# Jaakk0F/DSTD-GCN

Measured on AMD Instinct MI355X. Metric: pose-sequences/sec forward (H36M 22J×50T, B=256) at 1/2/4/8 GPUs; % HBM roofline, higher is better.
Workload: dtype f32; 1 GPU; H36M-shape synthetic, T=10+25=35, V=22, B=256/GPU, eval forward; global_batch=256, seq_len=35, joints=22, parallelism=dp1

## Files before the change

### dstd-gcn_amd/csrc/dstd_capi.hip

```cpp
#include <stdlib.h>
#include <string.h>

#include <algorithm>

#include <vector>

#include "../../include/dstd_gcn.h"
#include "../../include/dstd_gcn_taps.h"
#include "dstd_common.h"
#include "dstd_hilo.h"
#include "dstd_kernels.h"
#include "dstd_taps.h"

using namespace dstd;

namespace {

constexpr int kMaxT = 128;
constexpr int kMaxV = 32;
constexpr int kMaxC = 64;

struct Carver {
  char* base;
  size_t off = 0;
// ... 854 lines not shown
                        const dstd_block_taps* taps, void* workspace, size_t workspace_bytes, void* stream,
                        unsigned flags) {
  if ((flags & ~DSTD_FWD_EXACT_FP32) || !taps) return DSTD_EINVAL;
  return block_fwd(p, x, B, T, V, y, workspace, workspace_bytes, stream, flags, taps);
}

}

namespace {

int block_fwd(const dstd_block_params* p, const float* x, int B, int T, int V, float* y, void* workspace,
              size_t workspace_bytes, void* stream, unsigned flags, const dstd_block_taps* taps) {
  StreamDeviceGuard dev_guard_(stream, x);
  if (!x || !y || !workspace || !block_ok(p) || !shape_ok(B, T, V)) return DSTD_EINVAL;
  if (!limits_ok(T, V, p->cin, p->cout)) return DSTD_ELIMIT;
  if (workspace_bytes < dstd_block_workspace_bytes(B, p->cin, p->cout, T, V)) return DSTD_EWORKSPACE;
  hipStream_t s = (hipStream_t)stream;
  Carver cv{(char*)workspace};
  BlockLayout L;
  carve_block(cv, L, B, p->cin, p->cout, T, V);
  FoldList fa;
  add_block_jobs(fa, p, L.f, T, V);
  DSTD_TRY(run_fold(fa, s));
  DSTD_TRY(to_layout(x, L.xin, B, p->cin, T * V, 1, s));
  DSTD_TRY(spatial_pq(p, L.xin, B, T, V, L.sc.pq_s, s));
  BlockTail tail{TEPI_RAW, nullptr, nullptr, nullptr, nullptr, nullptr};
  const BlockHL hl = block_hl(p, tail, B, T, V, flags, taps != nullptr);
  HLList hj;
  add_block_hl_jobs(hj, p, L.f, tail, hl, T, V);
  DSTD_TRY(run_hl_prep(hj, s));
  Prof pf;
  DSTD_TRY(run_block(p, L.f, L.sc, B, T, V, L.xin, L.h, L.yout, tail, s, pf, hl, nullptr, taps));
  DSTD_TRY(to_layout(L.yout, y, B, p->cout, T * V, 0, s));
  return DSTD_OK;
}

}

extern "C" {

int dstd_model_fwd(const dstd_model_params* p, const float* x, int B, float* y, void* workspace,
                   size_t workspace_bytes, void* stream) {
  return dstd_model_fwd_ex(p, x, B, y, workspace, workspace_bytes, stream, 0u, nullptr);
}

int dstd_model_fwd_profiled(const dstd_model_params* p, const float* x, int B, float* y, void* workspace,
                            size_t workspace_bytes, void* stream, dstd_profile* prof) {
  return dstd_model_fwd_ex(p, x, B, y, workspace, workspace_bytes, stream, 0u, prof);
}

int dstd_model_fwd_ex(const dstd_model_params* p, const float* x, int B, float* y, void* workspace,
                      size_t workspace_bytes, void* stream, unsigned flags, dstd_profile* prof) {
  if (flags & ~(DSTD_FWD_REUSE_CONSTANTS | DSTD_FWD_EXACT_FP32 | DSTD_FWD_SEPARATE_ADJ | DSTD_FWD_FUSED_TEMPORAL |
                DSTD_FWD_SEPARATE_BLOCK | DSTD_FWD_SEPARATE_ENCODERS))
    return DSTD_EINVAL;
  return model_fwd(p, x, B, y, workspace, workspace_bytes, stream, flags, prof, nullptr);
}

size_t dstd_model_taps_workspace_bytes(int B, int T, int V, int num_feature, int num_layers) {
  return dstd_model_workspace_bytes(B, T, V, num_feature, num_layers);
}

int dstd_model_fwd_taps(const dstd_model_params* p, const float* x, int B, float* y, const dstd_block_taps* taps,
                        void* workspace, size_t workspace_bytes, void* stream, unsigned flags) {
  if ((flags & ~DSTD_FWD_EXACT_FP32) || !taps) return DSTD_EINVAL;
  return model_fwd(p, x, B, y, workspace, workspace_bytes, stream, flags, nullptr, taps);
}

}

namespace {

int model_fwd(const dstd_model_params* p, const float* x, int B, float* y, void* workspace, size_t workspace_bytes,
              void* stream, unsigned flags, dstd_profile* prof, const dstd_block_taps* taps) {
  StreamDeviceGuard dev_guard_(stream, x);
  if (taps) flags |= DSTD_FWD_SEPARATE_ADJ | DSTD_FWD_SEPARATE_BLOCK | DSTD_FWD_SEPARATE_ENCODERS;
  const bool reuse = (flags & DSTD_FWD_REUSE_CONSTANTS) != 0;
  if (!p || !x || !y || !workspace) return DSTD_EINVAL;
  if (prof && (prof->capacity < 0 || (prof->capacity > 0 && (!prof->events || !prof->kinds)))) return DSTD_EINVAL;
  Prof pf;
  pf.p = prof;
  const int T = p->T, V = p->V, C = p->num_feature, L_ = p->num_layers;
  if (!shape_ok(B, T, V) || L_ < 0 || L_ > DSTD_MAX_LAYERS || p->in_channels != 6) return DSTD_EINVAL;
  if (!limits_ok(T, V, p->in_channels, C)) return DSTD_ELIMIT;
  if (!block_ok(&p->st_in) || !block_ok(&p->st_out) || !bn_ok(p->bn_in) || !p->prelu) return DSTD_EINVAL;
  if (p->st_in.cin != 6 || p->st_in.cout != C || p->st_out.cin != C || p->st_out.cout != 3) return DSTD_EINVAL;
  for (int i = 0; i < L_; ++i) {
    if (!block_ok(&p->enc[i]) || !bn_ok(p->enc_bn[i]) || !p->enc_prelu[i]) return DSTD_EINVAL;
    if (p->enc[i].cin != C || p->enc[i].cout != C) return DSTD_EINVAL;
  }
  if (workspace_bytes < dstd_model_workspace_bytes(B, T, V, C, L_)) return DSTD_EWORKSPACE;
  hipStream_t s = (hipStream_t)stream;
  Carver cv{(char*)workspace};
  ModelLayout L;
  carve_model(cv, L, B, T, V, C, L_, 6, 3);

  FoldList fa;
  add_block_jobs(fa, &p->st_in, L.f_in, T, V);
  add_block_jobs(fa, &p->st_out, L.f_out, T, V);
  add_bn_job(fa, p->bn_in, C, V, L.bnin_s, L.bnin_h);
  for (int i = 0; i < L_; ++i) {
    add_block_jobs(fa, &p->enc[i], L.f_enc[i], T, V);
    add_bn_job(fa, p->enc_bn[i], C, V, L.ebn_s[i], L.ebn_h[i]);
  }
  if (!reuse) {
    pf.begin(DSTD_KIND_FOLD, s);
    DSTD_TRY(run_fold(fa, s));
// ... 44 lines not shown
    hls[b] = block_hl(blk[b], tails[b], B, T, V, flags, taps != nullptr);
    add_block_hl_jobs(hj, blk[b], *fold[b], tails[b], hls[b], T, V);
  }
  for (int b = 1; b < NB && !(flags & DSTD_FWD_SEPARATE_ADJ); ++b)
    if (hls[b].s && hls[b - 1].tf && blk[b - 1]->cout == 64 && temporal_fused_phase3(T, V)) {
      hls[b].s_pre = true;
      tails[b - 1].next_f = fold[b];
      tails[b - 1].next_adj = true;
    }
  if (hls[0].bf && !(flags & DSTD_FWD_SEPARATE_ADJ) && blk[0]->cin == 6 && block_fused_adj0_supported(T, V))
    hls[0].adj0 = true;

  PQArgs pa{};
  pa.x = x;
  pa.B = B;
  pa.T = T;
  pa.V = V;
  pa.Cin = 6;
  pa.make_x6 = 1;
  pa.x6 = L.act[0];
  const dstd_block_params* b0 = &p->st_in;
  pa.w[0] = b0->conv_s[0].wm1;
  pa.w[1] = b0->conv_s[0].wm2;
  pa.w[2] = b0->conv_s[1].wm1;
  pa.w[3] = b0->conv_s[1].wm2;
  pa.b[0] = b0->conv_s[0].bm1;
  pa.b[1] = b0->conv_s[0].bm2;
  pa.b[2] = b0->conv_s[1].bm1;
  pa.b[3] = b0->conv_s[1].bm2;
  pa.nw = 4;
  pa.pq = L.sc.pq_s;
  pa.pql = pq_layout_vt(8, T, V);
  if (!hls[0].s || (taps && taps[0].x)) {
    pf.begin(DSTD_KIND_PREP, s);
    DSTD_TRY(launch_pq(pa, s));
    pf.end(s);
  }

  if (!reuse) {
    pf.begin(DSTD_KIND_FOLD, s);
    DSTD_TRY(run_hl_prep(hj, s));
    pf.end(s);
  }
  const bool chain = !(flags & (DSTD_FWD_SEPARATE_ENCODERS | DSTD_FWD_SEPARATE_BLOCK | DSTD_FWD_SEPARATE_ADJ)) &&
                     !(prof && prof->capacity > 0) && enc_chain_supported(T, V);
  auto chain_block = [&](int b, EncChainArgs* c) {
    if (!chain || b < 1 || b > L_ || !hls[b].bf || !hls[b].s_pre || !tails[b].next_adj) return false;
    BlockArgs A;
    build_block_args(A, blk[b], *fold[b], L.sc, B, T, V, xin[b], hbuf[b], ybuf[b], tails[b], hls[b], nullptr);
    BlockFusedArgs ba;
    return block_fused_args(A.ha, A.ht, A.aht, &A.sn, &ba, nullptr) == hipSuccess &&
           enc_chain_append(c, ba) == hipSuccess;
  };
  for (int b = 0; b < NB;) {
    EncChainArgs c{};
    int e = b;
    while (e < NB && chain_block(e, &c)) ++e;
    if (e - b >= 2) {
      DSTD_TRY(launch_enc_chain(c, s));
      b = e;
      continue;
    }
    pf.block = b;
    DSTD_TRY(run_block(blk[b], *fold[b], L.sc, B, T, V, xin[b], hbuf[b], ybuf[b], tails[b], s, pf, hls[b],
                       b == 0 ? x : nullptr, taps ? &taps[b] : nullptr));
    ++b;
  }
  return DSTD_OK;
}

}

extern "C" {


int dstd_events_create(int n, void** events) {
  if (n < 0 || (n > 0 && !events)) return DSTD_EINVAL;
  for (int i = 0; i < n; ++i) {
    hipEvent_t e;
    DSTD_TRY(hipEventCreate(&e));
    events[i] = (void*)e;
  }
  return DSTD_OK;
}

int dstd_events_destroy(int n, void** events) {
  if (n < 0 || (n > 0 && !events)) return DSTD_EINVAL;
  for (int i = 0; i < n; ++i)
    if (events[i]) DSTD_TRY(hipEventDestroy((hipEvent_t)events[i]));
  return DSTD_OK;
}

int dstd_event_elapsed_ms(void* start, void* stop, float* ms) {
  if (!start || !stop || !ms) return DSTD_EINVAL;
  return (int)hipEventElapsedTime(ms, (hipEvent_t)start, (hipEvent_t)stop);
}

}
```

### dstd-gcn_amd/csrc/dstd_hilo.h

```cpp
#pragma once
#include "dstd_common.h"
#include "dstd_kernels.h"

namespace dstd {

typedef _Float16 f16x8 __attribute__((ext_vector_type(8)));

typedef float f32x2_t __attribute__((ext_vector_type(2)));
typedef _Float16 f16x2_t __attribute__((ext_vector_type(2)));

__device__ __forceinline__ void split8(const float4& a, const float4& b, uint4& hi, uint4& lo) {
  hi.x = __builtin_bit_cast(uint32_t, __builtin_convertvector((f32x2_t){a.x, a.y}, f16x2_t));
  hi.y = __builtin_bit_cast(uint32_t, __builtin_convertvector((f32x2_t){a.z, a.w}, f16x2_t));
  hi.z = __builtin_bit_cast(uint32_t, __builtin_convertvector((f32x2_t){b.x, b.y}, f16x2_t));
  hi.w = __builtin_bit_cast(uint32_t, __builtin_convertvector((f32x2_t){b.z, b.w}, f16x2_t));
  asm("v_fma_mixlo_f16 %0, %4, 1.0, -%12 op_sel_hi:[0,0,1]\n\t"
      "v_fma_mixhi_f16 %0, %5, 1.0, -%12 op_sel:[0,0,1] op_sel_hi:[0,0,1]\n\t"
      "v_fma_mixlo_f16 %1, %6, 1.0, -%13 op_sel_hi:[0,0,1]\n\t"
      "v_fma_mixhi_f16 %1, %7, 1.0, -%13 op_sel:[0,0,1] op_sel_hi:[0,0,1]\n\t"
      "v_fma_mixlo_f16 %2, %8, 1.0, -%14 op_sel_hi:[0,0,1]\n\t"
      "v_fma_mixhi_f16 %2, %9, 1.0, -%14 op_sel:[0,0,1] op_sel_hi:[0,0,1]\n\t"
      "v_fma_mixlo_f16 %3, %10, 1.0, -%15 op_sel_hi:[0,0,1]\n\t"
      "v_fma_mixhi_f16 %3, %11, 1.0, -%15 op_sel:[0,0,1] op_sel_hi:[0,0,1]\n\t"
      "s_nop 1"
// ... 259 lines not shown
};
static_assert(sizeof(EncChainArgs) <= 4096, "kernel arguments end at 4 KB");
__host__ __device__ inline void enc_chain_apply(const EncChainDesc& d, SpatialHLArgs& s) {
  s.x = d.x;
  s.y = d.h;
  for (int g = 0; g < 2; ++g) {
    s.wimg[g] = d.s_wimg[g];
    s.wscale[g] = d.s_wscale[g];
    s.bf[g] = d.s_bf[g];
    s.adjb[g] = d.s_adjb[g];
    s.pqb[g] = d.s_pqb[g];
  }
  s.bn_s = d.s_bn_s;
  s.bn_h = d.s_bn_h;
  s.prelu = d.s_prelu;
  s.pqimg = d.s_pqimg;
  s.pqscale = d.s_pqscale;
}
__host__ __device__ inline void enc_chain_apply(const EncChainDesc& d, TemporalHLArgs& g) {
  g.h = d.h;
  g.wimg = d.t_wimg;
  g.wscale = d.t_wscale;
  g.bf = d.t_bf;
  g.adjb = d.t_adjb;
  g.xres = d.t_xres;
  g.bn_s = d.t_bn_s;
  g.bn_h = d.t_bn_h;
  g.prelu = d.t_prelu;
  g.y = d.y;
  g.pqimg = d.t_pqimg;
  g.pqscale = d.t_pqscale;
  for (int i = 0; i < 4; ++i) g.pqb[i] = d.t_pqb[i];
}
__host__ __device__ inline void enc_chain_apply_j(const EncChainDesc& d, AdjHLArgs& j) {
  j.wimg[0] = d.j_wimg;
  j.wscale[0] = d.j_wscale;
  j.bias[0] = d.j_bias;
  j.astat[0] = d.j_astat;
  j.alpha = d.j_alpha;
}
__host__ __device__ inline void enc_chain_apply_sn(const EncChainDesc& d, AdjHLArgs& sn) {
  for (int g = 0; g < 2; ++g) {
    sn.wimg[g] = d.n_wimg[g];
    sn.wscale[g] = d.n_wscale[g];
    sn.bias[g] = d.n_bias[g];
    sn.astat[g] = d.n_astat[g];
  }
  sn.alpha = d.n_alpha;
}
bool enc_chain_supported(int T, int V);
hipError_t enc_chain_append(EncChainArgs* c, const BlockFusedArgs& a);
hipError_t launch_enc_chain(const EncChainArgs& c, hipStream_t s);


}
```

### dstd-gcn_amd/csrc/dstd_hilo.hip

```cpp
#include <type_traits>

#include "dstd_common.h"
#include "dstd_hilo.h"
#include "dstd_kernels.h"

#ifdef DSTD_STAMPS
__device__ unsigned long long g_tl_hl[6][2048][4];
#define TLH(m, i) \
  if (threadIdx.x == 0 && blockIdx.x < 2048) g_tl_hl[m][blockIdx.x][i] = __builtin_amdgcn_s_memrealtime();
#else
#define TLH(m, i)
#endif

namespace dstd {

namespace {


__device__ __forceinline__ float4 ld4(const float* p) { return *reinterpret_cast<const float4*>(p); }
__device__ __forceinline__ f16x8 as_h8(const uint4& v) { return __builtin_bit_cast(f16x8, v); }
typedef _Float16 f16x4 __attribute__((ext_vector_type(4)));

__device__ __forceinline__ f32x4 mfma32(const f16x8& a, const f16x8& b, f32x4 c) {
  return __builtin_amdgcn_mfma_f32_16x16x32_f16(a, b, c, 0, 0, 0);
// ... 2210 lines not shown
  __device__ __forceinline__ KP base() const {
    KP p = (KP)__builtin_amdgcn_kernarg_segment_ptr();
    asm volatile("" : "+s"(p));
    return p;
  }
  template <typename S, typename P>
  __device__ __forceinline__ static S get(P p) {
    S r;
    __builtin_memcpy(&r, p, sizeof(S));
    return r;
  }
  __device__ __forceinline__ SpatialHLArgsVal s() const {
    KP p = base();
    SpatialHLArgsVal r = get<SpatialHLArgsVal>(&p->s);
    enc_chain_apply(get<EncChainDesc>(&p->enc[b]), r);
    return r;
  }
  __device__ __forceinline__ TemporalHLArgs tg() const {
    KP p = base();
    TemporalHLArgs r = get<TemporalHLArgs>(&p->t.g);
    enc_chain_apply(get<EncChainDesc>(&p->enc[b]), r);
    return r;
  }
  __device__ __forceinline__ AdjHLArgs tj() const {
    KP p = base();
    AdjHLArgs r = get<AdjHLArgs>(&p->t.j);
    enc_chain_apply_j(get<EncChainDesc>(&p->enc[b]), r);
    return r;
  }
  __device__ __forceinline__ AdjHLArgs tsn() const {
    KP p = base();
    AdjHLArgs r = get<AdjHLArgs>(&p->t.sn);
    enc_chain_apply_sn(get<EncChainDesc>(&p->enc[b]), r);
    return r;
  }
  __device__ __forceinline__ AdjHLArgs s0() const { return AdjHLArgs{}; }
  __device__ __forceinline__ static uint32_t zero() { return (uint32_t)opaque_zero(); }
};

template <int T, int V>
__global__ __launch_bounds__((64 * tf_waves<T, V>())) __attribute__((amdgpu_waves_per_eu((tf_waves<T, V>() / 4), (tf_waves<T, V>() / 4)))) void k_enc_chain(EncChainArgs ca) {
  extern __shared__ __attribute__((aligned(16))) unsigned char dsm[];
#pragma nounroll
  for (int b = 0; b < ca.nblk; ++b) {
    int tid = threadIdx.x, n = blockIdx.x, lds0 = 0;
    asm volatile("" : "+v"(tid));
    asm volatile("" : "+s"(n), "+s"(lds0));
    block_fused_body<T, V, 64, 64, TEPI_ENC>(EncChainArgsAt{b}, n, dsm + lds0, tid);
    __builtin_amdgcn_s_waitcnt(0);
    __syncthreads();
  }
}

namespace {

int hl_num_cus() {
  static int n = [] {
    int dev = 0, v = 0;
    if (hipGetDevice(&dev) != hipSuccess ||
        hipDeviceGetAttribute(&v, hipDeviceAttributeMultiprocessorCount, dev) != hipSuccess || v <= 0)
      v = 256;
    return v;
  }();
  return n;
}

template <typename K>
int hl_occupancy(K k, int nt) {
  int nb = 0;
  if (hipOccupancyMaxActiveBlocksPerMultiprocessor(&nb, (const void*)k, nt, 0) != hipSuccess || nb < 1) nb = 1;
  (void)hipGetLastError();
  return nb;
}

template <auto K, int NT, typename A>
hipError_t launch_units(int units, const A& a, hipStream_t s) {
  static const int occ = hl_occupancy(K, NT);
  int grid = hl_num_cus() * occ;
  grid = min(grid, cdiv(units, NT / 64));
  hipLaunchKernelGGL(K, dim3(grid), dim3(NT), 0, s, a);
  return hipGetLastError();
}

template <int T>
hipError_t temporal_hl_t(const TemporalHLArgs& a, hipStream_t s) {
  if (a.C == 3) {
    if (a.pq) return hipErrorNotSupported;
    switch (a.epi) {
      case TEPI_OUT: return launch_units<k_temporal_hl<T, TEPI_OUT, 3>, temporal_nt<T, 3>()>(a.B * a.V, a, s);
      case TEPI_RAW: return launch_units<k_temporal_hl<T, TEPI_RAW, 3>, temporal_nt<T, 3>()>(a.B * a.V, a, s);
      default: return hipErrorNotSupported;
    }
  }
  if (a.C != 64) return hipErrorNotSupported;
  switch (a.epi) {
    case TEPI_ENC:
      if constexpr (tf_res_acc(T, 25)) {
        if (a.V == 25) return launch_units<k_temporal_hl<T, TEPI_ENC, 64, true>, temporal_nt<T, 64>()>(a.B * a.V, a, s);
      }
      if constexpr (tf_res_acc(T, 23)) {
        if (a.V == 23) return launch_units<k_temporal_hl<T, TEPI_ENC, 64, true>, temporal_nt<T, 64>()>(a.B * a.V, a, s);
      }
      return launch_units<k_temporal_hl<T, TEPI_ENC, 64>, temporal_nt<T, 64>()>(a.B * a.V, a, s);
    case TEPI_IN: return launch_units<k_temporal_hl<T, TEPI_IN, 64>, temporal_nt<T, 64>()>(a.B * a.V, a, s);
    case TEPI_RAW: return launch_units<k_temporal_hl<T, TEPI_RAW, 64>, temporal_nt<T, 64>()>(a.B * a.V, a, s);
    default: return hipErrorNotSupported;
// ... 109 lines not shown

template <int T, int V>
hipError_t bfused_tv(const BlockFusedArgs& a, hipStream_t s) {
  const int cin = a.s.Cin, cout = a.s.Cout, epi = a.t.g.epi;
  if (cin == 64 && cout == 64 && epi == TEPI_ENC) return bfused_run<T, V, 64, 64, TEPI_ENC>(a, s);
  if (cin == 6 && cout == 64 && epi == TEPI_IN) return bfused_run<T, V, 6, 64, TEPI_IN>(a, s);
  if (cin == 64 && cout == 3 && epi == TEPI_OUT) return bfused_run<T, V, 64, 3, TEPI_OUT>(a, s);
  return hipErrorNotSupported;
}

bool block_fused_supported(int T, int V, int cin, int cout, int epi) {
  const bool shape = (T == 35 && (V == 22 || V == 25)) || (T == 40 && V == 23);
  return shape && ((cin == 64 && cout == 64 && epi == TEPI_ENC) || (cin == 6 && cout == 64 && epi == TEPI_IN) ||
                   (cin == 64 && cout == 3 && epi == TEPI_OUT));
}

bool block_fused_adj0_supported(int T, int V) {
  return block_fused_supported(T, V, 6, 64, TEPI_IN) && temporal_fused_phase3(T, V);
}

static bool phase3_args_ok(const TemporalHLArgs& g, const AdjHLArgs& sn) {
  return temporal_fused_phase3(g.T, g.V) && g.C == 64 && g.pq && sn.pq == g.pq && sn.ngroups == 2 && !sn.xin &&
         sn.pql.sch == 1 && !(sn.pql.st & 3) && !(sn.pql.sv & 3) && !(sn.pql.sn & 3) && !(sn.p_ch[0] & 3) &&
         !(sn.p_ch[1] & 3) && sn.out;
}

hipError_t block_fused_args(const SpatialHLArgs& sa, const TemporalHLArgs& g, const AdjHLArgs& j, const AdjHLArgs* sn,
                            BlockFusedArgs* out, const AdjHLArgs* s0) {
  if (!block_fused_supported(g.T, g.V, sa.Cin, sa.Cout, g.epi) || sa.T != g.T || sa.V != g.V || sa.B != g.B ||
      sa.Cout != g.C || sa.y != g.h || sa.pq != j.pq || g.V != (int)(j.pql.st / 4) || j.pql.sch != 1 || j.pql.sv != 4 ||
      ((uintptr_t)j.pq & 15) || j.p_ch[0] != 0 || j.pql.sn != (long)g.T * g.V * 4)
    return hipErrorNotSupported;
  if (sn && !phase3_args_ok(g, *sn)) return hipErrorNotSupported;
  if (s0 && (sa.Cin != 6 || !block_fused_adj0_supported(g.T, g.V) || !s0->xin || s0->ngroups != 2 || !s0->out ||
             s0->B != g.B || !sa.xmodel || sa.adj != s0->out))
    return hipErrorNotSupported;
  *out = BlockFusedArgs{sa, TemporalFusedArgs{g, j, sn ? *sn : AdjHLArgs{}}, s0 ? *s0 : AdjHLArgs{}};
  return hipSuccess;
}

hipError_t launch_block_fused(const SpatialHLArgs& sa, const TemporalHLArgs& g, const AdjHLArgs& j, const AdjHLArgs* sn,
                              hipStream_t s, const AdjHLArgs* s0) {
  BlockFusedArgs a;
  const hipError_t e = block_fused_args(sa, g, j, sn, &a, s0);
  if (e != hipSuccess) return e;
  if (g.T == 35 && g.V == 22) return bfused_tv<35, 22>(a, s);
  if (g.T == 35 && g.V == 25) return bfused_tv<35, 25>(a, s);
  if (g.T == 40 && g.V == 23) return bfused_tv<40, 23>(a, s);
  return hipErrorNotSupported;
}

bool enc_chain_supported(int T, int V) { return block_fused_supported(T, V, 64, 64, TEPI_ENC) && temporal_fused_phase3(T, V); }

hipError_t enc_chain_append(EncChainArgs* c, const BlockFusedArgs& a) {
  const SpatialHLArgs& s = a.s;
  const TemporalHLArgs& g = a.t.g;
  const AdjHLArgs &j = a.t.j, &n = a.t.sn;
  if (!enc_chain_supported(g.T, g.V) || s.Cin != 64 || s.Cout != 64 || g.epi != TEPI_ENC || s.xmodel || !n.out ||
      a.s0.out || g.xres != s.x || s.wimg[2] || s.wscale[2] || s.bf[2] || s.rbn_s || s.rbn_h || j.xin || n.xin)
    return hipErrorNotSupported;
  if (c->nblk == 0) {
    c->s = s;
    c->t = a.t;
  } else {
    const SpatialHLArgs& s0 = c->s;
    const TemporalHLArgs& g0 = c->t.g;
    const AdjHLArgs &j0 = c->t.j, &n0 = c->t.sn;
    auto same_adj = [](const AdjHLArgs& p, const AdjHLArgs& q) {
      return p.pq == q.pq && p.pql.sn == q.pql.sn && p.pql.st == q.pql.st && p.pql.sv == q.pql.sv &&
             p.pql.sch == q.pql.sch && p.p_ch[0] == q.p_ch[0] && p.p_ch[1] == q.p_ch[1] && p.B == q.B &&
             p.ngroups == q.ngroups && p.out == q.out && p.out_sN == q.out_sN && p.out_sG == q.out_sG &&
             p.nchunk == q.nchunk;
    };
    if (c->nblk >= kEncChainMax || s.B != s0.B || s.T != s0.T || s.V != s0.V || s.adj != s0.adj || s.pq != s0.pq ||
        g.B != g0.B || g.T != g0.T || g.V != g0.V || g.C != g0.C || g.adj != g0.adj || g.pq != g0.pq ||
        !same_adj(j, j0) || !same_adj(n, n0))
      return hipErrorNotSupported;
  }
  EncChainDesc& d = c->enc[c->nblk++];
  d = EncChainDesc{};
  d.x = s.x;
  d.h = s.y;
  for (int i = 0; i < 2; ++i) {
    d.s_wimg[i] = s.wimg[i];
    d.s_wscale[i] = s.wscale[i];
    d.s_bf[i] = s.bf[i];
    d.s_adjb[i] = s.adjb[i];
    d.s_pqb[i] = s.pqb[i];
    d.n_wimg[i] = n.wimg[i];
    d.n_wscale[i] = n.wscale[i];
    d.n_bias[i] = n.bias[i];
    d.n_astat[i] = n.astat[i];
  }
  d.s_bn_s = s.bn_s;
  d.s_bn_h = s.bn_h;
  d.s_prelu = s.prelu;
  d.s_pqimg = s.pqimg;
  d.s_pqscale = s.pqscale;
  d.t_wimg = g.wimg;
  d.t_wscale = g.wscale;
  d.t_bf = g.bf;
  d.t_adjb = g.adjb;
  d.t_xres = g.xres;
  d.t_bn_s = g.bn_s;
  d.t_bn_h = g.bn_h;
  d.t_prelu = g.prelu;
  d.y = g.y;
  d.t_pqimg = g.pqimg;
  d.t_pqscale = g.pqscale;
  for (int i = 0; i < 4; ++i) d.t_pqb[i] = g.pqb[i];
  d.j_wimg = j.wimg[0];
  d.j_wscale = j.wscale[0];
  d.j_bias = j.bias[0];
  d.j_astat = j.astat[0];
  d.j_alpha = j.alpha;
  d.n_alpha = n.alpha;
  return hipSuccess;
}

template <int T, int V>
hipError_t enc_chain_run(const EncChainArgs& c, hipStream_t s) {
  using Gm = BlockFusedGeom<T, V, 64, 64, TEPI_ENC>;
  static const hipError_t attr = hipFuncSetAttribute((const void*)k_enc_chain<T, V>,
                                                     hipFuncAttributeMaxDynamicSharedMemorySize, (int)Gm::LDS);
  if (attr != hipSuccess) return attr;
  hipLaunchKernelGGL((k_enc_chain<T, V>), dim3(c.t.g.B), dim3(64 * tf_waves<T, V>()), Gm::LDS, s, c);
  return hipGetLastError();
}

hipError_t launch_enc_chain(const EncChainArgs& c, hipStream_t s) {
  if (c.nblk < 1 || c.nblk > kEncChainMax) return hipErrorInvalidValue;
  const int T = c.t.g.T, V = c.t.g.V;
  if (T == 35 && V == 22) return enc_chain_run<35, 22>(c, s);
  if (T == 35 && V == 25) return enc_chain_run<35, 25>(c, s);
  if (T == 40 && V == 23) return enc_chain_run<40, 23>(c, s);
  return hipErrorNotSupported;
}

bool temporal_fused_supported(int T, int V) {
  return (T == 35 && (V == 22 || V == 25)) || (T == 40 && V == 23) || (T == 75 && V == 22);
}
bool temporal_fused_default(int T, int V) {
  return temporal_fused_supported(T, V) && T != 75;
}
bool temporal_fused_phase3(int T, int V) {
  if (T == 35 && V == 22) return tf_phase3<35, 22>();
  if (T == 35 && V == 25) return tf_phase3<35, 25>();
  if (T == 40 && V == 23) return tf_phase3<40, 23>();
  if (T == 75 && V == 22) return tf_phase3<75, 22>();
  return false;
}

hipError_t launch_temporal_fused(const TemporalHLArgs& g, const AdjHLArgs& j, const AdjHLArgs* sn, hipStream_t s) {
  if (!temporal_fused_supported(g.T, g.V) || g.V != (int)(j.pql.st / 4) || j.pql.sch != 1 || j.pql.sv != 4 ||
      ((uintptr_t)j.pq & 15))
    return hipErrorNotSupported;
  if (sn && !phase3_args_ok(g, *sn)) return hipErrorNotSupported;
  const TemporalFusedArgs a{g, j, sn ? *sn : AdjHLArgs{}};
  if (g.T == 35 && g.V == 22) return tfused_tv<35, 22>(a, s);
  if (g.T == 35 && g.V == 25) return tfused_tv<35, 25>(a, s);
  if (g.T == 40 && g.V == 23) return tfused_tv<40, 23>(a, s);
  if (g.T == 75 && g.V == 22) return tfused_tv<75, 22>(a, s);
  return hipErrorNotSupported;
}

hipError_t launch_temporal_hl(const TemporalHLArgs& a, hipStream_t s) {
  if (!temporal_hl_supported(a.T, a.V)) return hipErrorNotSupported;
  switch (a.T) {
    case 35: return temporal_hl_t<35>(a, s);
    case 40: return temporal_hl_t<40>(a, s);
    case 75: return temporal_hl_t<75>(a, s);
    default: return hipErrorNotSupported;
  }
}

}

#ifdef DSTD_STAMPS
extern "C" int dstd_debug_timeline_hl(int mode, unsigned long long* host, int n) {
  if (mode < 0 || mode > 5 || n > 2048 * 4) return 1;
  return (int)hipMemcpyFromSymbol(host, HIP_SYMBOL(g_tl_hl), n * sizeof(unsigned long long),
                                  mode * 2048 * 4 * sizeof(unsigned long long));
}
#endif
```

### dstd-gcn_amd/dstd_native/__init__.py

```python
import ctypes
import os

import torch

_HERE = os.path.dirname(os.path.abspath(__file__))
LIB_PATH = os.environ.get("DSTD_LIB") or os.path.join(os.path.dirname(_HERE), "libdstd_gcn.so")

MODE_SPATIAL = 0
MODE_TEMPORAL = 1
MAX_LAYERS = 16

_fp = ctypes.POINTER(ctypes.c_float)


class GCWeights(ctypes.Structure):
    _fields_ = [(n, ctypes.c_void_p) for n in ("wf", "bf", "wm1", "bm1", "wm2", "bm2", "wrm", "brm")]


class BN(ctypes.Structure):
    _fields_ = [("weight", ctypes.c_void_p), ("bias", ctypes.c_void_p), ("running_mean", ctypes.c_void_p),
                ("running_var", ctypes.c_void_p), ("eps", ctypes.c_float)]


class BlockParams(ctypes.Structure):
# ... 25 lines not shown

TAP_NAMES = ("adj_s", "adj_t", "x", "h")


class GCGrads(ctypes.Structure):
    _fields_ = [(n, ctypes.c_void_p) for n in ("wf", "bf", "wm1", "bm1", "wm2", "bm2", "wrm", "brm")]


class BNGrads(ctypes.Structure):
    _fields_ = [("weight", ctypes.c_void_p), ("bias", ctypes.c_void_p)]


class BlockGrads(ctypes.Structure):
    _fields_ = [("W_s", ctypes.c_void_p), ("R_s", ctypes.c_void_p), ("R_t", ctypes.c_void_p),
                ("alpha_sm", ctypes.c_void_p), ("alpha_tm", ctypes.c_void_p),
                ("conv_s", GCGrads * 2), ("conv_t", GCGrads), ("bn", BNGrads), ("prelu", ctypes.c_void_p),
                ("res_w", ctypes.c_void_p), ("res_b", ctypes.c_void_p), ("res_bn", BNGrads)]


class ModelGrads(ctypes.Structure):
    _fields_ = [("st_in", BlockGrads), ("bn_in", BNGrads), ("prelu", ctypes.c_void_p),
                ("enc", BlockGrads * MAX_LAYERS), ("enc_bn", BNGrads * MAX_LAYERS),
                ("enc_prelu", ctypes.c_void_p * MAX_LAYERS), ("st_out", BlockGrads)]


COLL_ALLGATHER, COLL_ALLREDUCE_SUM = 0, 1
COLLECTIVE_FN = ctypes.CFUNCTYPE(ctypes.c_int, ctypes.c_void_p, ctypes.c_int, ctypes.c_void_p, ctypes.c_longlong,
                                 ctypes.c_void_p)


class BnSyncStruct(ctypes.Structure):
    _fields_ = [("world", ctypes.c_int), ("rank", ctypes.c_int), ("fn", COLLECTIVE_FN), ("ctx", ctypes.c_void_p),
                ("buf", ctypes.c_void_p), ("buf_floats", ctypes.c_longlong)]


class LossProblem(ctypes.Structure):
    _fields_ = [("pred", ctypes.c_void_p), ("targ", ctypes.c_void_p), ("B", ctypes.c_int), ("T", ctypes.c_int),
                ("V", ctypes.c_int), ("targ_T", ctypes.c_int), ("targ_t0", ctypes.c_int), ("targ_step", ctypes.c_int)]


LOSS_JL2, LOSS_TL2, LOSS_CL1, LOSS_CL2 = 1, 2, 4, 8
LOSS_NTERMS = 4

TRAIN_RUNNING_STATS = 1
TRAIN_PAIRED = 2
TRAIN_SEED_DEVICE = 4
TRAIN_ONE_STREAM = 8
FWD_REUSE_CONSTANTS = 1
FWD_EXACT_FP32 = 2
FWD_SEPARATE_ADJ = 4
FWD_FUSED_TEMPORAL = 8
FWD_SEPARATE_BLOCK = 16
FWD_SEPARATE_ENCODERS = 32
KIND_FOLD, KIND_PREP, KIND_ADJ_S, KIND_SPATIAL, KIND_ADJ_T, KIND_TEMPORAL, KIND_BLOCK = range(7)
KIND_NAMES = ("fold", "prep", "adj_spatial", "spatial_gc", "adj_temporal", "temporal_gc", "block")

_lib = None


def source_hash():
    import glob
    import hashlib
    pkg = os.path.dirname(_HERE)
    rel = [os.path.relpath(p, pkg) for pat in ("csrc/*.hip", "csrc/*.h", "../include/*.h")
           for p in glob.glob(os.path.join(pkg, pat))]
    files = sorted(rel) + ["Makefile"]
    h = hashlib.sha256()
    for f in files:
        path = os.path.join(pkg, f)
        if not os.path.exists(path):
            return None
        with open(path, "rb") as fh:
            h.update(fh.read())
    return h.hexdigest()[:16]


def lib():
    global _lib
    if _lib is None:
        if not os.path.exists(LIB_PATH):
            raise RuntimeError(f"DSTD native library not built: {LIB_PATH} (run `make -C dstd-gcn_amd`)")
        L = ctypes.CDLL(LIB_PATH)
        vp, sz, ci = ctypes.c_void_p, ctypes.c_size_t, ctypes.c_int
        L.dstd_source_hash.restype = ctypes.c_char_p
        built, tree = L.dstd_source_hash().decode(), source_hash()
        if tree is not None and built != tree and os.environ.get("DSTD_AB_FOREIGN_LIB") != "1":
            raise RuntimeError(f"{LIB_PATH} was built from other sources (hash {built}, this tree {tree}): "
                               "rebuild with `make -C dstd-gcn_amd`")
        L.dstd_version.restype = ctypes.c_char_p
        L.dstd_error_string.restype = ctypes.c_char_p
        L.dstd_error_string.argtypes = [ci]
        L.dstd_dstdgc_workspace_bytes.restype = sz
        L.dstd_dstdgc_workspace_bytes.argtypes = [ci] * 6
        L.dstd_block_workspace_bytes.restype = sz
        L.dstd_block_workspace_bytes.argtypes = [ci] * 5
        L.dstd_model_workspace_bytes.restype = sz
        L.dstd_model_workspace_bytes.argtypes = [ci] * 5
        L.dstd_dstdgc_fwd.restype = ci
        L.dstd_dstdgc_fwd.argtypes = [ci, vp, ci, ci, ci, ci, ci, ctypes.POINTER(GCWeights), vp, vp, vp, vp, sz, vp]
        L.dstd_block_fwd.restype = ci
        L.dstd_block_fwd.argtypes = [ctypes.POINTER(BlockParams), vp, ci, ci, ci, vp, vp, sz, vp]
        L.dstd_block_fwd_ex.restype = ci
        L.dstd_block_fwd_ex.argtypes = [ctypes.POINTER(BlockParams), vp, ci, ci, ci, vp, vp, sz, vp, ctypes.c_uint]
        L.dstd_model_fwd.restype = ci
        L.dstd_model_fwd.argtypes = [ctypes.POINTER(ModelParams), vp, ci, vp, vp, sz, vp]
        L.dstd_model_fwd_ex.restype = ci
# ... 286 lines not shown
```

### include/dstd_gcn.h

```cpp
#ifndef DSTD_GCN_H
#define DSTD_GCN_H

#include <stddef.h>

#ifdef __cplusplus
extern "C" {
#endif

#define DSTD_OK 0
#define DSTD_EINVAL -1
#define DSTD_EWORKSPACE -2
#define DSTD_ELIMIT -3
#define DSTD_ECOLLECTIVE -5

#define DSTD_MODE_SPATIAL 0
#define DSTD_MODE_TEMPORAL 1
#define DSTD_MAX_LAYERS 16

typedef struct dstd_gc_weights {
  const float* wf;
  const float* bf;
  const float* wm1;
  const float* bm1;
  const float* wm2;
// ... 37 lines not shown
  dstd_bn enc_bn[DSTD_MAX_LAYERS];
  const float* enc_prelu[DSTD_MAX_LAYERS];
  dstd_block_params st_out;
} dstd_model_params;

const char* dstd_version(void);
const char* dstd_source_hash(void);
const char* dstd_error_string(int code);

size_t dstd_dstdgc_workspace_bytes(int mode, int B, int cin, int cout, int T, int V);
size_t dstd_block_workspace_bytes(int B, int cin, int cout, int T, int V);
size_t dstd_model_workspace_bytes(int B, int T, int V, int num_feature, int num_layers);

int dstd_dstdgc_fwd(int mode, const float* x, int B, int cin, int cout, int T, int V,
                    const dstd_gc_weights* w, const float* A, const float* alpha, float* y,
                    void* workspace, size_t workspace_bytes, void* stream);

int dstd_block_fwd(const dstd_block_params* p, const float* x, int B, int T, int V, float* y,
                   void* workspace, size_t workspace_bytes, void* stream);
int dstd_block_fwd_ex(const dstd_block_params* p, const float* x, int B, int T, int V, float* y,
                      void* workspace, size_t workspace_bytes, void* stream, unsigned flags);

int dstd_model_fwd(const dstd_model_params* p, const float* x, int B, float* y, void* workspace,
                   size_t workspace_bytes, void* stream);

#define DSTD_KIND_FOLD 0
#define DSTD_KIND_PREP 1
#define DSTD_KIND_ADJ_S 2
#define DSTD_KIND_SPATIAL 3
#define DSTD_KIND_ADJ_T 4
#define DSTD_KIND_TEMPORAL 5
#define DSTD_KIND_BLOCK 6
#define DSTD_KIND_COUNT 7

typedef struct dstd_profile {
  unsigned kind_mask;
  int capacity;
  int count;
  void** events;
  int* kinds;
  int* block;
  int only_block;
} dstd_profile;

int dstd_model_fwd_profiled(const dstd_model_params* p, const float* x, int B, float* y, void* workspace,
                            size_t workspace_bytes, void* stream, dstd_profile* prof);

#define DSTD_FWD_REUSE_CONSTANTS 1u
#define DSTD_FWD_EXACT_FP32 2u
#define DSTD_FWD_SEPARATE_ADJ 4u
#define DSTD_FWD_FUSED_TEMPORAL 8u
#define DSTD_FWD_SEPARATE_BLOCK 16u
#define DSTD_FWD_SEPARATE_ENCODERS 32u
int dstd_model_fwd_ex(const dstd_model_params* p, const float* x, int B, float* y, void* workspace,
                      size_t workspace_bytes, void* stream, unsigned flags, dstd_profile* prof);
int dstd_events_create(int n, void** events);
int dstd_events_destroy(int n, void** events);
int dstd_event_elapsed_ms(void* start, void* stop, float* ms);


#ifdef __cplusplus
}
#endif
#endif
```

Measured before the change: 476,700 seq/s.

## Fuse input, encoder and output blocks into one persistent model-chain kernel

Adds a k_model_chain kernel that runs the input block (with its adjacency prep), all encoder blocks, and the output block in one launch, with per-CTA sync between phases, instead of launching the input and output blocks separately around the encoder chain. The goal is to remove kernel launch overhead and inter-kernel gaps across the whole forward. The kernel argument struct grows toward the 4 KB limit, and the LDS is sized for the largest phase. A new flag DSTD_FWD_SEPARATE_ENDS restores the old path.

```diff
diff --git a/dstd-gcn_amd/csrc/dstd_capi.hip b/dstd-gcn_amd/csrc/dstd_capi.hip
--- a/dstd-gcn_amd/csrc/dstd_capi.hip
+++ b/dstd-gcn_amd/csrc/dstd_capi.hip
@@ -930,7 +930,7 @@
 int dstd_model_fwd_ex(const dstd_model_params* p, const float* x, int B, float* y, void* workspace,
                       size_t workspace_bytes, void* stream, unsigned flags, dstd_profile* prof) {
   if (flags & ~(DSTD_FWD_REUSE_CONSTANTS | DSTD_FWD_EXACT_FP32 | DSTD_FWD_SEPARATE_ADJ | DSTD_FWD_FUSED_TEMPORAL |
-                DSTD_FWD_SEPARATE_BLOCK | DSTD_FWD_SEPARATE_ENCODERS))
+                DSTD_FWD_SEPARATE_BLOCK | DSTD_FWD_SEPARATE_ENCODERS | DSTD_FWD_SEPARATE_ENDS))
     return DSTD_EINVAL;
   return model_fwd(p, x, B, y, workspace, workspace_bytes, stream, flags, prof, nullptr);
 }
@@ -1081,6 +1081,33 @@
     return block_fused_args(A.ha, A.ht, A.aht, &A.sn, &ba, nullptr) == hipSuccess &&
            enc_chain_append(c, ba) == hipSuccess;
   };
+  auto model_chain = [&](ModelChainArgs* c) {
+    if (!chain || (flags & DSTD_FWD_SEPARATE_ENDS) || taps || L_ < 1 || L_ > kModelChainMaxEnc ||
+        !model_chain_supported(T, V) || !hls[0].bf || !hls[0].adj0 || !tails[0].next_adj || !hls[NB - 1].bf ||
+        !hls[NB - 1].s_pre)
+      return false;
+    for (int b = 1; b <= L_; ++b)
+      if (!hls[b].bf || !hls[b].s_pre || !tails[b].next_adj) return false;
+    for (int i = 0; i < NB; ++i) {
+      const int b = i < L_ ? 1 + i : i == L_ ? 0 : NB - 1;
+      float* hb = b == NB - 1 ? L.sc.adj_t : hbuf[b];
+      BlockArgs A;
+      build_block_args(A, blk[b], *fold[b], L.sc, B, T, V, xin[b], hb, ybuf[b], tails[b], hls[b], b == 0 ? x : nullptr);
+      BlockFusedArgs ba;
+      if (block_fused_args(A.ha, A.ht, A.aht, tails[b].next_adj ? &A.sn : nullptr, &ba,
+                           b == 0 && A.from_model ? &A.ah : nullptr) != hipSuccess ||
+          model_chain_append(c, ba) != hipSuccess)
+        return false;
+    }
+    return model_chain_complete(*c);
+  };
+  {
+    ModelChainArgs mc{};
+    if (model_chain(&mc)) {
+      DSTD_TRY(launch_model_chain(mc, s));
+      return DSTD_OK;
+    }
+  }
   for (int b = 0; b < NB;) {
     EncChainArgs c{};
     int e = b;
diff --git a/dstd-gcn_amd/csrc/dstd_hilo.h b/dstd-gcn_amd/csrc/dstd_hilo.h
--- a/dstd-gcn_amd/csrc/dstd_hilo.h
+++ b/dstd-gcn_amd/csrc/dstd_hilo.h
@@ -335,5 +335,81 @@
 hipError_t enc_chain_append(EncChainArgs* c, const BlockFusedArgs& a);
 hipError_t launch_enc_chain(const EncChainArgs& c, hipStream_t s);
 
-
-}
+struct ModelEndDesc {
+  EncChainDesc e;
+  const uint4* s_wimg2;
+  const float* s_wscale2;
+  const float* s_bf2;
+  const float* s_rbn_s;
+  const float* s_rbn_h;
+};
+struct ModelAdj0Desc {
+  const float* xin;
+  const float* mw[2][2];
+  const float* mb[2][2];
+  const uint4* wimg[2];
+  const float* wscale[2];
+  const float* bias[2];
+  const float* astat[2];
+  const float* alpha;
+};
+constexpr int kModelChainMaxEnc = 5;
+struct ModelChainArgs {
+  SpatialHLArgs s;
+  TemporalFusedArgs t;
+  int nenc;
+  int have;
+  EncChainDesc enc[kModelChainMaxEnc];
+  ModelEndDesc in, out;
+  ModelAdj0Desc in0;
+};
+static_assert(sizeof(ModelChainArgs) + 256 <= 4096, "kernel arguments (with the hidden ones) end at 4 KB");
+__host__ __device__ inline void model_chain_apply_res(const ModelEndDesc& d, SpatialHLArgs& s) {
+  s.wimg[2] = d.s_wimg2;
+  s.wscale[2] = d.s_wscale2;
+  s.bf[2] = d.s_bf2;
+  s.rbn_s = d.s_rbn_s;
+  s.rbn_h = d.s_rbn_h;
+}
+__host__ __device__ inline void model_chain_apply_in(const ModelEndDesc& d, SpatialHLArgs& s) {
+  enc_chain_apply(d.e, s);
+  model_chain_apply_res(d, s);
+  s.xmodel = 1;
+  s.Cin = 6;
+}
+__host__ __device__ inline void model_chain_apply_in(const ModelEndDesc& d, TemporalHLArgs& g) {
+  enc_chain_apply(d.e, g);
+  g.epi = TEPI_IN;
+}
+__host__ __device__ inline void model_chain_apply_in0(const ModelAdj0Desc& d, AdjHLArgs& s0) {
+  s0.xin = d.xin;
+  for (int g = 0; g < 2; ++g) {
+    for (int i = 0; i < 2; ++i) {
+      s0.mw[g][i] = d.mw[g][i];
+      s0.mb[g][i] = d.mb[g][i];
+    }
+    s0.wimg[g] = d.wimg[g];
+    s0.wscale[g] = d.wscale[g];
+    s0.bias[g] = d.bias[g];
+    s0.astat[g] = d.astat[g];
+  }
+  s0.alpha = d.alpha;
+}
+__host__ __device__ inline void model_chain_apply_out(const ModelEndDesc& d, SpatialHLArgs& s) {
+  enc_chain_apply(d.e, s);
+  model_chain_apply_res(d, s);
+  s.Cout = 3;
+}
+__host__ __device__ inline void model_chain_apply_out(const ModelEndDesc& d, TemporalHLArgs& g) {
+  enc_chain_apply(d.e, g);
+  g.C = 3;
+  g.epi = TEPI_OUT;
+  g.pq = nullptr;
+}
+bool model_chain_supported(int T, int V);
+hipError_t model_chain_append(ModelChainArgs* c, const BlockFusedArgs& a);
+bool model_chain_complete(const ModelChainArgs& c);
+hipError_t launch_model_chain(const ModelChainArgs& c, hipStream_t s);
+
+
+}
diff --git a/dstd-gcn_amd/csrc/dstd_hilo.hip b/dstd-gcn_amd/csrc/dstd_hilo.hip
--- a/dstd-gcn_amd/csrc/dstd_hilo.hip
+++ b/dstd-gcn_amd/csrc/dstd_hilo.hip
@@ -2286,6 +2286,103 @@
   }
 }
 
+template <int PH>
+struct ModelChainArgsAt {
+  int b;
+  typedef const ModelChainArgs __attribute__((address_space(4))) * KP;
+  __device__ __forceinline__ KP base() const {
+    KP p = (KP)__builtin_amdgcn_kernarg_segment_ptr();
+    asm volatile("" : "+s"(p));
+    return p;
+  }
+  template <typename S, typename P>
+  __device__ __forceinline__ static S get(P p) {
+    S r;
+    __builtin_memcpy(&r, p, sizeof(S));
+    return r;
+  }
+  __device__ __forceinline__ SpatialHLArgsVal s() const {
+    KP p = base();
+    SpatialHLArgsVal r = get<SpatialHLArgsVal>(&p->s);
+    if constexpr (PH == 0) model_chain_apply_in(get<ModelEndDesc>(&p->in), r);
+    else if constexpr (PH == 1) enc_chain_apply(get<EncChainDesc>(&p->enc[b]), r);
+    else model_chain_apply_out(get<ModelEndDesc>(&p->out), r);
+    return r;
+  }
+  __device__ __forceinline__ TemporalHLArgs tg() const {
+    KP p = base();
+    TemporalHLArgs r = get<TemporalHLArgs>(&p->t.g);
+    if constexpr (PH == 0) model_chain_apply_in(get<ModelEndDesc>(&p->in), r);
+    else if constexpr (PH == 1) enc_chain_apply(get<EncChainDesc>(&p->enc[b]), r);
+    else model_chain_apply_out(get<ModelEndDesc>(&p->out), r);
+    return r;
+  }
+  __device__ __forceinline__ EncChainDesc desc(KP p) const {
+    if constexpr (PH == 0) return get<EncChainDesc>(&p->in.e);
+    else if constexpr (PH == 1) return get<EncChainDesc>(&p->enc[b]);
+    else return get<EncChainDesc>(&p->out.e);
+  }
+  __device__ __forceinline__ AdjHLArgs tj() const {
+    KP p = base();
+    AdjHLArgs r = get<AdjHLArgs>(&p->t.j);
+    enc_chain_apply_j(desc(p), r);
+    return r;
+  }
+  __device__ __forceinline__ AdjHLArgs tsn() const {
+    KP p = base();
+    AdjHLArgs r = get<AdjHLArgs>(&p->t.sn);
+    enc_chain_apply_sn(desc(p), r);
+    return r;
+  }
+  __device__ __forceinline__ AdjHLArgs s0() const {
+    if constexpr (PH != 0) return AdjHLArgs{};
+    KP p = base();
+    AdjHLArgs r = get<AdjHLArgs>(&p->t.sn);
+    model_chain_apply_in0(get<ModelAdj0Desc>(&p->in0), r);
+    return r;
+  }
+  __device__ __forceinline__ static uint32_t zero() { return PH == 0 ? 0u : (uint32_t)opaque_zero(); }
+};
+
+template <int T, int V>
+struct ModelChainGeom {
+  static constexpr size_t LI = BlockFusedGeom<T, V, 6, 64, TEPI_IN>::LDS, LE = BlockFusedGeom<T, V, 64, 64, TEPI_ENC>::LDS,
+                          LO = BlockFusedGeom<T, V, 64, 3, TEPI_OUT>::LDS;
+  static constexpr size_t LDS = LI > LE ? (LI > LO ? LI : LO) : (LE > LO ? LE : LO);
+};
+
+#define DSTD_CHAIN_OPAQUE_IDS                      \
+  int tid = threadIdx.x, n = blockIdx.x, lds0 = 0; \
+  asm volatile("" : "+v"(tid));                    \
+  asm volatile("" : "+s"(n), "+s"(lds0));
+#define DSTD_CHAIN_BOUNDARY          \
+  __builtin_amdgcn_s_waitcnt(0);     \
+  __syncthreads();
+
+template <int T, int V>
+__global__ __launch_bounds__((64 * tf_waves<T, V>())) __attribute__((amdgpu_waves_per_eu((tf_waves<T, V>() / 4), (tf_waves<T, V>() / 4)))) void k_model_chain(ModelChainArgs ca) {
+  extern __shared__ __attribute__((aligned(16))) unsigned char dsm[];
+  {
+    const unsigned idy = __builtin_amdgcn_workitem_id_y(), idz = __builtin_amdgcn_workitem_id_z();
+    __builtin_assume(idy == 0);
+    __builtin_assume(idz == 0);
+    block_fused_body<T, V, 6, 64, TEPI_IN>(ModelChainArgsAt<0>{0}, blockIdx.x, dsm, threadIdx.x);
+    DSTD_CHAIN_BOUNDARY
+  }
+#pragma nounroll
+  for (int b = 0; b < ca.nenc; ++b) {
+    DSTD_CHAIN_OPAQUE_IDS
+    block_fused_body<T, V, 64, 64, TEPI_ENC>(ModelChainArgsAt<1>{b}, n, dsm + lds0, tid);
+    DSTD_CHAIN_BOUNDARY
+  }
+  {
+    DSTD_CHAIN_OPAQUE_IDS
+    block_fused_body<T, V, 64, 3, TEPI_OUT>(ModelChainArgsAt<2>{0}, n, dsm + lds0, tid);
+  }
+}
+#undef DSTD_CHAIN_OPAQUE_IDS
+#undef DSTD_CHAIN_BOUNDARY
+
 namespace {
 
 int hl_num_cus() {
@@ -2501,33 +2598,45 @@
 
 bool enc_chain_supported(int T, int V) { return block_fused_supported(T, V, 64, 64, TEPI_ENC) && temporal_fused_phase3(T, V); }
 
-hipError_t enc_chain_append(EncChainArgs* c, const BlockFusedArgs& a) {
+static bool enc_chain_kind_ok(const BlockFusedArgs& a) {
   const SpatialHLArgs& s = a.s;
   const TemporalHLArgs& g = a.t.g;
   const AdjHLArgs &j = a.t.j, &n = a.t.sn;
-  if (!enc_chain_supported(g.T, g.V) || s.Cin != 64 || s.Cout != 64 || g.epi != TEPI_ENC || s.xmodel || !n.out ||
-      a.s0.out || g.xres != s.x || s.wimg[2] || s.wscale[2] || s.bf[2] || s.rbn_s || s.rbn_h || j.xin || n.xin)
+  return enc_chain_supported(g.T, g.V) && s.Cin == 64 && s.Cout == 64 && g.epi == TEPI_ENC && !s.xmodel && n.out &&
+         !a.s0.out && g.xres == s.x && !s.wimg[2] && !s.wscale[2] && !s.bf[2] && !s.rbn_s && !s.rbn_h && !j.xin && !n.xin;
+}
+static bool chain_same_adj(const AdjHLArgs& p, const AdjHLArgs& q) {
+  return p.pq == q.pq && p.pql.sn == q.pql.sn && p.pql.st == q.pql.st && p.pql.sv == q.pql.sv &&
+         p.pql.sch == q.pql.sch && p.p_ch[0] == q.p_ch[0] && p.p_ch[1] == q.p_ch[1] && p.B == q.B &&
+         p.ngroups == q.ngroups && p.out == q.out && p.out_sN == q.out_sN && p.out_sG == q.out_sG &&
+         p.nchunk == q.nchunk;
+}
+static bool enc_chain_same_geometry(const BlockFusedArgs& a, const SpatialHLArgs& s0, const TemporalFusedArgs& t0) {
+  const SpatialHLArgs& s = a.s;
+  const TemporalHLArgs &g = a.t.g, &g0 = t0.g;
+  return s.B == s0.B && s.T == s0.T && s.V == s0.V && s.adj == s0.adj && s.pq == s0.pq && g.B == g0.B && g.T == g0.T &&
+         g.V == g0.V && g.C == g0.C && g.adj == g0.adj && g.pq == g0.pq && chain_same_adj(a.t.j, t0.j) &&
+         chain_same_adj(a.t.sn, t0.sn);
+}
+static EncChainDesc enc_chain_desc(const BlockFusedArgs& a);
+
+hipError_t enc_chain_append(EncChainArgs* c, const BlockFusedArgs& a) {
+  if (!enc_chain_kind_ok(a)) return hipErrorNotSupported;
+  if (c->nblk == 0) {
+    c->s = a.s;
+    c->t = a.t;
+  } else if (c->nblk >= kEncChainMax || !enc_chain_same_geometry(a, c->s, c->t)) {
     return hipErrorNotSupported;
-  if (c->nblk == 0) {
-    c->s = s;
-    c->t = a.t;
-  } else {
-    const SpatialHLArgs& s0 = c->s;
-    const TemporalHLArgs& g0 = c->t.g;
-    const AdjHLArgs &j0 = c->t.j, &n0 = c->t.sn;
-    auto same_adj = [](const AdjHLArgs& p, const AdjHLArgs& q) {
-      return p.pq == q.pq && p.pql.sn == q.pql.sn && p.pql.st == q.pql.st && p.pql.sv == q.pql.sv &&
-             p.pql.sch == q.pql.sch && p.p_ch[0] == q.p_ch[0] && p.p_ch[1] == q.p_ch[1] && p.B == q.B &&
-             p.ngroups == q.ngroups && p.out == q.out && p.out_sN == q.out_sN && p.out_sG == q.out_sG &&
-             p.nchunk == q.nchunk;
-    };
-    if (c->nblk >= kEncChainMax || s.B != s0.B || s.T != s0.T || s.V != s0.V || s.adj != s0.adj || s.pq != s0.pq ||
-        g.B != g0.B || g.T != g0.T || g.V != g0.V || g.C != g0.C || g.adj != g0.adj || g.pq != g0.pq ||
-        !same_adj(j, j0) || !same_adj(n, n0))
-      return hipErrorNotSupported;
-  }
-  EncChainDesc& d = c->enc[c->nblk++];
-  d = EncChainDesc{};
+  }
+  c->enc[c->nblk++] = enc_chain_desc(a);
+  return hipSuccess;
+}
+
+static EncChainDesc enc_chain_desc(const BlockFusedArgs& a) {
+  const SpatialHLArgs& s = a.s;
+  const TemporalHLArgs& g = a.t.g;
+  const AdjHLArgs &j = a.t.j, &n = a.t.sn;
+  EncChainDesc d{};
   d.x = s.x;
   d.h = s.y;
   for (int i = 0; i < 2; ++i) {
@@ -2564,7 +2673,7 @@
   d.j_astat = j.astat[0];
   d.j_alpha = j.alpha;
   d.n_alpha = n.alpha;
-  return hipSuccess;
+  return d;
 }
 
 template <int T, int V>
@@ -2583,6 +2692,95 @@
   if (T == 35 && V == 22) return enc_chain_run<35, 22>(c, s);
   if (T == 35 && V == 25) return enc_chain_run<35, 25>(c, s);
   if (T == 40 && V == 23) return enc_chain_run<40, 23>(c, s);
+  return hipErrorNotSupported;
+}
+
+bool model_chain_supported(int T, int V) {
+  return enc_chain_supported(T, V) && block_fused_adj0_supported(T, V) && block_fused_supported(T, V, 64, 3, TEPI_OUT);
+}
+
+bool model_chain_complete(const ModelChainArgs& c) { return c.nenc >= 1 && c.have == 3; }
+
+hipError_t model_chain_append(ModelChainArgs* c, const BlockFusedArgs& a) {
+  const SpatialHLArgs& s = a.s;
+  const TemporalHLArgs& g = a.t.g;
+  const AdjHLArgs &j = a.t.j, &n = a.t.sn;
+  if (!model_chain_supported(g.T, g.V)) return hipErrorNotSupported;
+  const bool enc = s.Cin == 64 && s.Cout == 64 && g.epi == TEPI_ENC;
+  const bool in = s.Cin == 6 && s.Cout == 64 && g.epi == TEPI_IN, out = s.Cin == 64 && s.Cout == 3 && g.epi == TEPI_OUT;
+  if (enc) {
+    if (c->have || c->nenc >= kModelChainMaxEnc || !enc_chain_kind_ok(a)) return hipErrorNotSupported;
+    if (c->nenc == 0) {
+      c->s = s;
+      c->t = a.t;
+    } else if (!enc_chain_same_geometry(a, c->s, c->t)) {
+      return hipErrorNotSupported;
+    }
+    c->enc[c->nenc++] = enc_chain_desc(a);
+    return hipSuccess;
+  }
+  if (!(in || out) || c->nenc < 1 || (c->have & (in ? 1 : 2))) return hipErrorNotSupported;
+  const SpatialHLArgs& sg = c->s;
+  const TemporalHLArgs& gg = c->t.g;
+  const AdjHLArgs &jg = c->t.j, &ng = c->t.sn;
+  if (s.B != sg.B || s.T != sg.T || s.V != sg.V || s.adj != sg.adj || s.pq != sg.pq || g.B != gg.B || g.T != gg.T ||
+      g.V != gg.V || g.adj != gg.adj || !chain_same_adj(j, jg) || j.xin || !s.wimg[2] || !s.wscale[2] || !s.bf[2] ||
+      !s.rbn_s || !s.rbn_h)
+    return hipErrorNotSupported;
+  if (in) {
+    const AdjHLArgs& z = a.s0;
+    if (!s.xmodel || g.C != gg.C || g.pq != gg.pq || g.xres || !n.out || n.xin || !chain_same_adj(n, ng) || !z.out ||
+        z.xin != s.x || !chain_same_adj(z, ng))
+      return hipErrorNotSupported;
+  } else {
+    if (s.xmodel || g.C != 3 || g.pq || g.pqimg || g.pqscale || n.out || a.s0.out || !g.xres)
+      return hipErrorNotSupported;
+  }
+  ModelEndDesc& d = in ? c->in : c->out;
+  d = ModelEndDesc{};
+  d.e = enc_chain_desc(a);
+  d.s_wimg2 = s.wimg[2];
+  d.s_wscale2 = s.wscale[2];
+  d.s_bf2 = s.bf[2];
+  d.s_rbn_s = s.rbn_s;
+  d.s_rbn_h = s.rbn_h;
+  if (in) {
+    const AdjHLArgs& z = a.s0;
+    ModelAdj0Desc& q = c->in0;
+    q = ModelAdj0Desc{};
+    q.xin = z.xin;
+    for (int i = 0; i < 2; ++i) {
+      for (int k = 0; k < 2; ++k) {
+        q.mw[i][k] = z.mw[i][k];
+        q.mb[i][k] = z.mb[i][k];
+      }
+      q.wimg[i] = z.wimg[i];
+      q.wscale[i] = z.wscale[i];
+      q.bias[i] = z.bias[i];
+      q.astat[i] = z.astat[i];
+    }
+    q.alpha = z.alpha;
+  }
+  c->have |= in ? 1 : 2;
+  return hipSuccess;
+}
+
+template <int T, int V>
+hipError_t model_chain_run(const ModelChainArgs& c, hipStream_t s) {
+  using Gm = ModelChainGeom<T, V>;
+  static const hipError_t attr = hipFuncSetAttribute((const void*)k_model_chain<T, V>,
+                                                     hipFuncAttributeMaxDynamicSharedMemorySize, (int)Gm::LDS);
+  if (attr != hipSuccess) return attr;
+  hipLaunchKernelGGL((k_model_chain<T, V>), dim3(c.t.g.B), dim3(64 * tf_waves<T, V>()), Gm::LDS, s, c);
+  return hipGetLastError();
+}
+
+hipError_t launch_model_chain(const ModelChainArgs& c, hipStream_t s) {
+  if (!model_chain_complete(c) || c.nenc > kModelChainMaxEnc) return hipErrorInvalidValue;
+  const int T = c.t.g.T, V = c.t.g.V;
+  if (T == 35 && V == 22) return model_chain_run<35, 22>(c, s);
+  if (T == 35 && V == 25) return model_chain_run<35, 25>(c, s);
+  if (T == 40 && V == 23) return model_chain_run<40, 23>(c, s);
   return hipErrorNotSupported;
 }
 
diff --git a/dstd-gcn_amd/dstd_native/__init__.py b/dstd-gcn_amd/dstd_native/__init__.py
--- a/dstd-gcn_amd/dstd_native/__init__.py
+++ b/dstd-gcn_amd/dstd_native/__init__.py
@@ -101,6 +101,7 @@
 FWD_FUSED_TEMPORAL = 8
 FWD_SEPARATE_BLOCK = 16
 FWD_SEPARATE_ENCODERS = 32
+FWD_SEPARATE_ENDS = 64
 KIND_FOLD, KIND_PREP, KIND_ADJ_S, KIND_SPATIAL, KIND_ADJ_T, KIND_TEMPORAL, KIND_BLOCK = range(7)
 KIND_NAMES = ("fold", "prep", "adj_spatial", "spatial_gc", "adj_temporal", "temporal_gc", "block")
 
diff --git a/include/dstd_gcn.h b/include/dstd_gcn.h
--- a/include/dstd_gcn.h
+++ b/include/dstd_gcn.h
@@ -113,6 +113,7 @@
 #define DSTD_FWD_FUSED_TEMPORAL 8u
 #define DSTD_FWD_SEPARATE_BLOCK 16u
 #define DSTD_FWD_SEPARATE_ENCODERS 32u
+#define DSTD_FWD_SEPARATE_ENDS 64u
 int dstd_model_fwd_ex(const dstd_model_params* p, const float* x, int B, float* y, void* workspace,
                       size_t workspace_bytes, void* stream, unsigned flags, dstd_profile* prof);
 int dstd_events_create(int n, void** events);
```

New measurement: 495,000 seq/s, median of 6. 3.8% higher.
